# sdat2/mSWE-GNN

Measured on AMD Instinct MI355X. Metric: mesh-nodes x rollout-steps / sec (fine-scale nodes); fp32 max-abs err vs CPU ref, higher is better.
Workload: dtype f32

## Files before the change

mswe-gnn_amd/csrc/engine.h:

```cpp
#pragma once
#include <hip/hip_runtime.h>
#include <stdint.h>
#include <algorithm>

#include "graph_build.h"

namespace msw {

constexpr int kMaxLayers = 4;
constexpr int kWaves = 4;
constexpr int kRowsPerBlock = kRowsPerWave * kWaves;
constexpr int kXcds = 8, kCusPerXcd = 32;

struct LayerDev {
  int tin, tout;
  int a_off, b_off;
  int act;
  float slope;
};
struct MlpDev {
  int n;
  LayerDev l[kMaxLayers];
};

// ... 121 lines not shown
  const float* skip;
  float* out;
  int last;
  Epilogue epi;
  int coop;
  int stagger;
  int wdirect;
  int* step_inc;
  const EdgeChunk* chunks; int nchunks;
  PoolFuse pool;
};

struct HopArgs {
  Common c;
  WReg reg;
  int max_blocks;
  int fit_blocks;
  int n0;
  const LaneRec* recs; int ntiles;
  const float* s;
  const float* xs;
  const float* in;
  float* out;
  int filt_a;
  int grad, upwind;
  int last;
  Epilogue epi;
  int coop;
  int split;
  int rows;
  int nrows;
  const int* rptr;
  const int2* redge;
};


struct PoolArgs {
  Common c;
  WReg reg;
  int max_blocks;
  int fit_blocks;
  int n0, ns;
  int rows;
  int ntiles;
  const PoolRec* recs;
  const LaneRec* erecs;
  int rtiles, etiles;
  const int* child;
  const float* in;
  const float* xs;
  NpDesc np;
  int coop;
};

struct EpiArgs {
  Common c;
  WReg reg;
  int max_blocks, fit_blocks;
  int n0, ns, ntiles;
  const float* in;
  const float* xs;
  float* out;
  Epilogue epi;
};

struct DecodeArgs {
  Common c;
// ... 30 lines not shown
constexpr size_t eh_lds_bytes(int floats) {
  return (size_t)((floats + kChunk - 1) / kChunk * kChunk) * sizeof(float);
}
template <int NT>
constexpr int edge_coop_lds_cap(int pw, int fuse) {
  if constexpr (NT == 4) {
    return 160 * 1024 - (kWaves / pw) * (kRowsPerWave * (48 * NT + 4) * 4 + 2 * kRowsPerWave * (32 * NT + 4) * 4);
  } else {
    const int st = kWaves * kRowsPerWave * (48 * NT + 4) * 4 + (kWaves / 2) * 2 * kRowsPerWave * (32 * NT + 4) * 4;
    const int ps = fuse ? (kWaves / 2) * kRowsPerWave * (48 * NT + 4) * 4 : 0;
    return 160 * 1024 - st - ps;
  }
}
int set_error(int code, const char* msg);

hipError_t launch_set_slots(const SlotArgs& a, hipStream_t st);
hipError_t launch_set_io(RolloutIO* dst, const RolloutIO& v, hipStream_t st);
hipError_t launch_init_state(const InitArgs& a, hipStream_t st);
hipError_t launch_copy_rows(const float* src, const int* srows, float* dst, const int* drows, int n, int width,
                            hipStream_t st);

struct Pick {
  const void* fn;
  char name[40];
  int err;
  int grid;
  int waves;
  int pack;
  size_t lds;
  long units;
  int per_wg;
};

static inline int cdiv(long a, long b) { return (int)((a + b - 1) / b); }

template <class A>
static inline bool tile_loop(const A& a) {
  return a.fit_blocks > 0 && a.max_blocks > 0 && cdiv(a.ntiles, kWaves) > a.fit_blocks;
}

template <class A>
static inline dim3 xcd_grid(A& b, long g) {
  b.c.xcd = 0;
  for (int k = 1; k <= b.c.xcd_max && k < kXcds; k *= 2)
    if (g <= (long)kCusPerXcd * k) {
      b.c.xcd = k;
      return dim3((unsigned)(cdiv(g, k) * kXcds));
    }
  return dim3((unsigned)g);
}

template <class A>
static inline hipError_t launch_pick(const Pick& p, const A& a, hipStream_t st) {
  if (p.err) return (hipError_t)p.err;
  if (!p.fn) return hipSuccess;
  A b = a;
  const dim3 grid = p.pack ? xcd_grid(b, p.grid) : dim3((unsigned)p.grid);
  if (!p.pack) b.c.xcd = 0;
  void* args[] = {&b};
  return hipLaunchKernel(p.fn, grid, dim3(64 * p.waves), args, p.lds, st);
}

enum Family { K_ENCODE, K_ENCODE_COOP, K_EDGE_HOP, K_EDGE_COOP, K_EDGE_MLP, K_HOP, K_HOP_ROWS, K_HOP_SPLIT,
              K_HOP_COOP, K_POOL_ROWS, K_POOL_EDGE, K_EPI, K_DECODE, K_FAMILIES };
struct VariantKey {
  int family;
  int prelu = 0;
  int last = 0;
  int loop = 0;
  int waves = 0;
  int fuse = 0;
  int dec = 0;
  int stream = 0;
};

template <int NT> Pick pick_encode(const EncodeArgs& a);
template <int NT> Pick pick_edge_hop(const EdgeHopArgs& a);
template <int NT> Pick pick_edge_mlp(const EdgeHopArgs& a);
template <int NT> Pick pick_hop(const HopArgs& a);
template <int NT> Pick pick_pool(const PoolArgs& a);
template <int NT> Pick pick_epi(const EpiArgs& a);
template <int NT> Pick pick_decode(const DecodeArgs& a);
template <int NT> hipError_t prepare_kernels();
template <int NT> int resident_blocks(const VariantKey& k, int floats);
template <int NT> hipError_t launch_rowmlp(const RowMlpArgs& a, hipStream_t st);

}
```

mswe-gnn_amd/csrc/graph_build.h:

```cpp
#pragma once
#include <stdint.h>

#include <algorithm>
#include <string>
#include <vector>

#include "../../include/mswegnn.h"
#include "tiling.h"

namespace msw {

constexpr int kRowsPerWave = 16;
constexpr int kMaxScales = 8;
constexpr int kPoolInline = 4;

struct I2 {
  int x, y;
};

struct TileRange {
  int node0, nnode, edge0, nedge;
};
struct LaneRec {
  int src;
// ... 18 lines not shown
  int ntiles = 0, nchunks = 0;
  std::vector<LaneRec> recs;
  std::vector<EdgeChunk> chunks;
  std::vector<int> porig;
  std::vector<int> rptr;
  std::vector<I2> redge;
};
struct HostLevel {
  int I = 0;
  std::vector<PoolRec> pool_recs;
  std::vector<LaneRec> pool_erecs;
  int pool_etiles = 0;
  std::vector<int> pool_child;
  std::vector<PoolSlot> pool_slots;
  std::vector<LaneRec> un_recs;
  int un_ntiles = 0;
  std::vector<I2> parent_slots;
};
struct HostGraph {
  int N = 0, Npad = 0;
  int64_t E = 0;
  std::vector<int> perm, iperm;
  std::vector<HostScale> sc;
  std::vector<HostLevel> lv;
};

struct XchPeer {
  int peer, roff, rcount, soff, scount;
};
struct HostXchScale {
  std::vector<int> recv_rows, send_rows;
  std::vector<XchPeer> peers;
};

inline void csr_build(int nkeys, const std::vector<int>& key, std::vector<int>& rowptr, std::vector<int>& order) {
  rowptr.assign(nkeys + 1, 0);
  for (int k : key) rowptr[k + 1]++;
  for (int i = 0; i < nkeys; ++i) rowptr[i + 1] += rowptr[i];
  std::vector<int> pos(rowptr.begin(), rowptr.end() - 1);
  order.assign(key.size(), 0);
  for (size_t e = 0; e < key.size(); ++e) order[pos[key[e]]++] = (int)e;
}

inline int build_tiles(const std::vector<int>& rowptr, std::vector<TileRange>& out, std::string& err) {
  out.clear();
  const int ns = (int)rowptr.size() - 1;
  int a = 0;
  while (a < ns) {
    int b = a, edges = 0;
    while (b < ns && b - a < kRowsPerWave) {
      const int d = rowptr[b + 1] - rowptr[b];
      if (d > kRowsPerWave) {
        err = "node with more than 16 in-edges";
        return MSW_ERR_UNSUPPORTED;
      }
      if (edges + d > kRowsPerWave) break;
      edges += d;
      ++b;
    }
    out.push_back(TileRange{a, b - a, rowptr[a], edges});
    a = b;
  }
  return MSW_OK;
}

inline std::vector<LaneRec> make_recs(const std::vector<int>& rowptr, const std::vector<int>& src, int n0,
// ... 258 lines not shown
```

mswe-gnn_amd/csrc/kernels/k_hop.h:

```cpp
#pragma once

template <int NT>
struct HopRows {
  Lanes L;
  f32x4 os[NT], sv[NT], inn[NT];
  EpiPre<NT> pre;
};
template <int NT, bool LAST>
__device__ __forceinline__ void hop_gather(HopRows<NT>& r, const HopArgs& a, const LaneRec& rec, int tile, int j,
                                           int g) {
  constexpr int F = 16 * NT;
  r.L = lanes_of(rec, tile, j, a.n0);
  load_row<NT>(r.os, a.in + r.L.sr * F, g);
  load_row<NT>(r.sv, a.s + r.L.p * F, g);
  load_row<NT>(r.inn, a.in + r.L.n * F, g);
  if constexpr (LAST) epi_prefetch<NT>(r.pre, a.epi, a.c, a.xs, r.L.n, g);
}
template <int NT, bool LAST>
__device__ __forceinline__ void hop_load(HopRows<NT>& r, const HopArgs& a, int tile, int j, int g) {
  hop_gather<NT, LAST>(r, a, load_rec(a.recs, tile, j), tile, j, g);
}
#define MSW_ARGS_HOP(a) \
  (a).c.xcd, (a).ntiles, (a).recs, (a).n0, (a).in, (a).s, (a).out, (a).c.W, (a).filt_a, (a).grad, (a).upwind
#define MSW_ARGS_HOP_LAST(a) \
// ... 86 lines not shown
      int t1 = tile + stride;
      LaneRec rn = load_rec(a.recs, t1 < a.ntiles ? t1 : tile, j);
      for (;;) {
        const int ln = opaque_lane(), gg = ln >> 4, jj = ln & 15;
        const bool more = t1 < a.ntiles;
        HopRows<NT> qn;
        if (more) {
          hop_gather<NT, LAST>(qn, a, rn, t1, jj, gg);
          const int t2 = t1 + stride;
          rn = load_rec(a.recs, t2 < a.ntiles ? t2 : t1, jj);
        }
        f32x4 res[NT];
        core(q, jj, ln, gg, res);
        finish(res, q, ln, gg);
        if (!more) break;
        q = qn;
        t1 += stride;
      }
    }
  }
  MSW_MARK(c, 9);
}

constexpr int kRowHopWaves = 8;
constexpr int kRowDc = 3;
template <int NT>
__global__ __launch_bounds__(64 * kRowHopWaves) void k_hop_rows(HopArgs a) {
#pragma clang fp contract(off)
  constexpr int F = 16 * NT;
  constexpr int DC = NT >= 4 ? 2 : kRowDc;
  [[maybe_unused]] const int lane = threadIdx.x & 63;
  const int w = wave_id();
  const int stride = gridDim.x * kRowHopWaves;
  MSW_PIN(stride, a.nrows, a.rptr, a.redge, a.n0, a.in, a.s, a.out, a.c.W, a.filt_a, a.grad, a.upwind);
  const int ntile = (a.nrows + kRowsPerWave - 1) / kRowsPerWave;
  f32x4 wf[NT][NT];
  load_filter<NT>(wf, a.c.W, a.filt_a, lane);
  for (int tile = blockIdx.x * kRowHopWaves + w; tile < ntile; tile += stride) {
    const int ln = opaque_lane(), g = ln >> 4, j = ln & 15;
    const int k = tile * kRowsPerWave + j;
    const bool valid = k < a.nrows;
    const int kc = valid ? k : 0;
    const int q0 = a.rptr[kc], q1 = valid ? a.rptr[kc + 1] : q0;
    const size_t n = (size_t)a.n0 + kc;
    f32x4 od[NT];
    load_row<NT>(od, a.in + n * F, g);
    const int deg = q1 - q0;
    int dmax = deg;
#pragma unroll
    for (int o = 1; o < 64; o <<= 1) dmax = max(dmax, __shfl_xor(dmax, o));
    float rd = 0.f;
#pragma unroll
    for (int t = 0; t < NT; ++t) rd += hsum(od[t]);
    const bool zd = row_sum(rd) != 0.f;
    f32x4 agg[NT];
#pragma unroll
    for (int t = 0; t < NT; ++t) agg[t] = zero4();
    for (int q = 0; q < dmax; q += DC) {
      int2 e[DC];
#pragma unroll
      for (int u = 0; u < DC; ++u)
        e[u] = q + u < deg ? a.redge[q0 + q + u] : int2{(int)n, 0};
      f32x4 os[DC][NT], sv[DC][NT];
#pragma unroll
      for (int u = 0; u < DC; ++u) {
        load_row<NT>(os[u], a.in + (size_t)e[u].x * F, g);
        load_row<NT>(sv[u], a.s + (size_t)e[u].y * F, g);
      }
#pragma unroll
      for (int u = 0; u < DC; ++u) {
        float rs = 0.f;
#pragma unroll
        for (int t = 0; t < NT; ++t) rs += hsum(os[u][t]);
        const bool act = (row_sum(rs) != 0.f) || zd;
        const bool has = q + u < deg;
#pragma unroll
        for (int t = 0; t < NT; ++t) {
          f32x4 gv;
          if (a.grad) {
            gv = od[t] - os[u][t];
            if (a.upwind) {
              gv.x = gv.x < 0.f ? 0.f : gv.x; gv.y = gv.y < 0.f ? 0.f : gv.y;
              gv.z = gv.z < 0.f ? 0.f : gv.z; gv.w = gv.w < 0.f ? 0.f : gv.w;
            }
          } else {
            gv = os[u][t];
          }
          const f32x4 m = act ? gv * sv[u][t] : zero4();
          const f32x4 sum = agg[t] + m;
          agg[t] = has ? sum : agg[t];
        }
      }
    }
    f32x4 res[NT];
#pragma unroll
    for (int t = 0; t < NT; ++t) res[t] = od[t];
    apply_filter_regs<NT>(res, agg, a.filt_a, wf);
    if (valid) store_row<NT, true>(a.out + n * F, res, NT, g);
  }
}

template <int NT>
__global__ __launch_bounds__(kBlock) void k_hop_split(HopArgs a) {
#pragma clang fp contract(off)
  constexpr int F = 16 * NT, TH = NT / 2, G = kWaves / 2;
  constexpr int XS = 16 * TH + 4;
  __shared__ __attribute__((aligned(16))) float slab_all[G][2][kRowsPerWave][XS];
  __shared__ __attribute__((aligned(16))) float hx[G][2][2 * TH][64];
  __shared__ __attribute__((aligned(16))) f32x4 ax[G][NT][64];
  const int lane = threadIdx.x & 63, g = lane >> 4, j = lane & 15, w = wave_id();
  const int grp = w / 2, r = w % 2, t0 = r * TH;
  MSW_PIN(MSW_ARGS_HOP(a));
  const int xb = logical_block(a.c);
  if (xb < 0) return;
  const int tile = xb * G + grp;
  const bool live = tile < a.ntiles;
  MSW_MARK(a.c, 0);
  const Lanes L = lanes_of(load_rec(a.recs, live ? tile : 0, j), live ? tile : 0, j, a.n0);
  f32x4 os[TH], sv[TH], inn[TH];
#pragma unroll
  for (int t = 0; t < TH; ++t) {
    const int off = 16 * (t0 + t) + 4 * g;
    os[t] = ld4(a.in + L.sr * F + off);
    sv[t] = ld4(a.s + L.p * F + off);
    inn[t] = ld4(a.in + L.n * F + off);
  }
  f32x4 wf[TH][NT];
  {
    const int fa = a.filt_a >= 0 ? a.filt_a : 0;
#pragma unroll
    for (int to = 0; to < TH; ++to)
#pragma unroll
// ... 206 lines not shown
```

mswe-gnn_amd/csrc/kernels/k_launch.h:

```cpp
#pragma once

template <int NT>
hipError_t prepare_kernels() {
  std::set<const void*> done;
  hipError_t e = hipSuccess;
  for_each_key([&](const VariantKey& k) {
    const Variant v = variant_of<NT>(k);
    if (e == hipSuccess && v.fn && v.lds_cap && done.insert(v.fn).second)
      e = hipFuncSetAttribute(v.fn, hipFuncAttributeMaxDynamicSharedMemorySize, v.lds_cap);
  });
  return e;
}

template <int NT>
hipError_t launch_rowmlp(const RowMlpArgs& a, hipStream_t st) {
  if (a.R <= 0) return hipSuccess;
  if (a.mode == 1)
    hipLaunchKernelGGL((k_rowmlp<NT, 1>), dim3(cdiv(a.R, kRowsPerBlock)), dim3(kBlock), 0, st, a);
  else
    hipLaunchKernelGGL((k_rowmlp<NT, 0>), dim3(cdiv(a.R, kRowsPerBlock)), dim3(kBlock), 0, st, a);
  return hipGetLastError();
}

template <int NT>
int resident_blocks(const VariantKey& k, int floats) {
  const Variant v = variant_of<NT>(k);
  int per_cu = 0, dev = 0, cus = 0;
  if (!v.fn) return 0;
  const size_t dyn = variant_lds<NT>(v, floats);
  if (dyn > 160 * 1024) return 0;
  if (hipOccupancyMaxActiveBlocksPerMultiprocessor(&per_cu, v.fn, 64 * v.waves, dyn) != hipSuccess)
    return 0;
  if (hipGetDevice(&dev) != hipSuccess || hipDeviceGetAttribute(&cus, hipDeviceAttributeMultiprocessorCount, dev) != hipSuccess)
    return 0;
  return per_cu > 0 ? per_cu * cus : 0;
}

#define MSW_INSTANTIATE(NT)                                                       \
  template hipError_t prepare_kernels<NT>();                                      \
  template int resident_blocks<NT>(const VariantKey&, int);                       \
  template Pick pick_encode<NT>(const EncodeArgs&);                               \
  template Pick pick_edge_hop<NT>(const EdgeHopArgs&);                            \
  template Pick pick_edge_mlp<NT>(const EdgeHopArgs&);                            \
  template Pick pick_hop<NT>(const HopArgs&);                                     \
  template Pick pick_pool<NT>(const PoolArgs&);                                   \
  template Pick pick_epi<NT>(const EpiArgs&);                                     \
  template Pick pick_decode<NT>(const DecodeArgs&);                               \
  template hipError_t launch_rowmlp<NT>(const RowMlpArgs&, hipStream_t);
```

mswe-gnn_amd/csrc/kernels/k_pick.h:

```cpp
#pragma once

template <int NT>
constexpr size_t lds_bytes(int floats) {
  return kStaged<NT> ? (size_t)((floats + kChunk - 1) / kChunk * kChunk) * sizeof(float) : 0;
}

template <class A>
static inline int tile_grid(const A& a) {
  return tile_loop(a) ? a.max_blocks : cdiv(a.ntiles, kWaves);
}

enum LdsRule { LDS_NONE, LDS_STAGED, LDS_EDGE_HOP };
struct Variant {
  const void* fn;
  int waves;
  int lds;
  int lds_cap;
};
template <int NT>
static inline size_t variant_lds(const Variant& v, int floats) {
  return v.lds == LDS_EDGE_HOP ? eh_lds_bytes(floats) : v.lds == LDS_STAGED ? lds_bytes<NT>(floats) : 0;
}

template <class F>
// ... 21 lines not shown
            k.dec ? act((const void*)k_encode_coop<NT, 1, true, NT>, (const void*)k_encode_coop<NT, -1, true, NT>)
                  : act((const void*)k_encode_coop<NT, 1, false, NT>, (const void*)k_encode_coop<NT, -1, false, NT>);
        return {f, enc_coop_waves<NT>(), LDS_STAGED, mx(enc_coop_waves<NT>())};
      }
      return none;
    case K_EDGE_HOP:
      return by_flag(k.loop, [&](auto lp) {
        return by_flag(k.last, [&](auto ls) {
          constexpr bool L = decltype(lp)::value;
          constexpr int LS = decltype(ls)::value;
          return Variant{act((const void*)k_edge_hop<NT, 1, L, LS>, (const void*)k_edge_hop<NT, -1, L, LS>),
                         edge_waves<NT, L, LS>(), LDS_EDGE_HOP, mx(edge_waves<NT, L, LS>())};
        });
      });
    case K_EDGE_COOP: {
      if (k.waves != 2 && !(NT == 4 && k.waves == 4)) return none;
      const void* f = edge_coop_kernel<NT>(k.prelu, k.last, k.waves, k.fuse);
      return {f, kWaves, LDS_EDGE_HOP, f ? edge_coop_lds_cap<NT>(k.waves, k.fuse) : 0};
    }
    case K_EDGE_MLP:
      return {act((const void*)k_edge_mlp<NT, 1>, (const void*)k_edge_mlp<NT, -1>), kMlpWaves, LDS_EDGE_HOP, 160 * 1024};
    case K_HOP:
      return by_flag(k.loop, [&](auto lp) {
        constexpr bool L = decltype(lp)::value;
        const void* f = !k.last ? (const void*)k_hop<NT, 1, false, L>
                                : act((const void*)k_hop<NT, 1, true, L>, (const void*)k_hop<NT, -1, true, L>);
        return Variant{f, hop_waves<NT, L>(), LDS_STAGED, k.last ? mx(hop_waves<NT, L>()) : 0};
      });
    case K_HOP_ROWS: return {(const void*)k_hop_rows<NT>, kRowHopWaves, LDS_NONE, 0};
    case K_HOP_SPLIT:
      if constexpr (NT >= 2) return {(const void*)k_hop_split<NT>, kWaves, LDS_NONE, 0};
      return none;
    case K_HOP_COOP: return {hop_coop_kernel<NT>(k.prelu), kWaves, LDS_STAGED, mx(kWaves)};
    case K_POOL_ROWS:
      return by_flag(k.loop, [&](auto lp) {
        constexpr bool L = decltype(lp)::value;
        return Variant{(const void*)k_pool<NT, L>, waves_of<NT, L>(), LDS_STAGED, mx(waves_of<NT, L>())};
      });
    case K_POOL_EDGE:
      if (k.waves <= 1) return {(const void*)k_pool_edge<NT>, kWaves, LDS_STAGED, mx(kWaves)};
      if constexpr (NT >= 2) {
        if (k.waves == NT) return {(const void*)k_pool_edge<NT, NT>, kWaves, LDS_STAGED, mx(kWaves)};
        if (k.waves == 2 * NT) return {(const void*)k_pool_edge<NT, 2 * NT, 2 * NT>, 2 * NT, LDS_STAGED, mx(2 * NT)};
      }
      return none;
    case K_EPI:
      return by_flag(k.loop, [&](auto lp) {
        constexpr bool L = decltype(lp)::value;
        return Variant{act((const void*)k_epi<NT, 1, L>, (const void*)k_epi<NT, -1, L>), waves_of<NT, L>(), LDS_STAGED,
                       mx(waves_of<NT, L>())};
      });
    case K_DECODE:
      return {act((const void*)k_decode_fwd<NT, 1>, (const void*)k_decode_fwd<NT, -1>), kWaves, LDS_NONE, 0};
  }
  return none;
}

template <class F>
static inline void for_each_key(F&& f) {
  for (int family = 0; family < K_FAMILIES; ++family)
    for (int bits = 0; bits < 32; ++bits)
      for (int waves : {1, 2, 4, 8})
        for (int fuse = 0; fuse < 3; ++fuse)
          f(VariantKey{family, bits & 1, bits >> 1 & 1, bits >> 2 & 1, waves, fuse, bits >> 3 & 1, bits >> 4 & 1});
}

// ... 64 lines not shown
                         a.ntiles, kWaves / a.coop);
  }
  if (a.pool.slots || a.pool.parent) return pick_invalid();
  const bool loop = tile_loop(a);
  const Variant v = variant_of<NT>({K_EDGE_HOP, a.c.prelu, a.last, loop});
  return pick_make<NT>(v, pick_name(nm, "edge_hop", {{loop, "loop"}, {last, "last"}, {!last, "first"}}), tile_grid(a),
                       !loop, loop ? a.reg.len : a.reg_nf, a.ntiles, v.waves);
}

template <int NT>
Pick pick_hop(const HopArgs& a) {
  if (a.ntiles <= 0) return Pick{};
  char nm[40];
  if (a.coop > 1 && a.last)
    return pick_make<NT>(variant_of<NT>({K_HOP_COOP, a.c.prelu, 1, 0, a.coop}), "hop coop",
                         cdiv((long)a.ntiles * a.coop, kWaves), 1, a.reg.len, a.ntiles, kWaves / a.coop);
  if (a.rows && !a.last) {
    const int nt = cdiv(a.nrows, kRowsPerWave);
    const int grid = a.max_blocks > 0 ? std::min(a.max_blocks, cdiv(nt, kRowHopWaves)) : cdiv(nt, kRowHopWaves);
    return pick_make<NT>(variant_of<NT>({K_HOP_ROWS}), "hop rows", grid, 0, 0, nt, kRowHopWaves);
  }
  if constexpr (NT >= 2) {
    if (a.split && !a.last)
      return pick_make<NT>(variant_of<NT>({K_HOP_SPLIT}), "hop split", cdiv((long)a.ntiles * 2, kWaves), 1, 0,
                           a.ntiles, kWaves / 2);
  }
  const bool loop = tile_loop(a), last = a.last != 0;
  const Variant v = variant_of<NT>({K_HOP, a.c.prelu, last, loop});
  return pick_make<NT>(v, pick_name(nm, "hop", {{loop, "loop"}, {last, "last"}, {!last, "mid"}}), tile_grid(a), !loop,
                       last ? a.reg.len : 0, a.ntiles, v.waves);
}

template <int NT>
Pick pick_pool(const PoolArgs& a) {
  if (a.ntiles <= 0) return Pick{};
  if (!a.rows) {
    if constexpr (NT >= 2) {
      if (a.coop == 2 * NT)
        return pick_make<NT>(variant_of<NT>({K_POOL_EDGE, 0, 0, 0, 2 * NT}), "pool edge wide", a.ntiles, 1, a.reg.len,
                             a.ntiles, 1);
      if (a.coop == NT)
        return pick_make<NT>(variant_of<NT>({K_POOL_EDGE, 0, 0, 0, NT}), "pool edge coop",
                             cdiv((long)a.ntiles * NT, kWaves), 1, a.reg.len, a.ntiles, kWaves / NT);
    }
    return pick_make<NT>(variant_of<NT>({K_POOL_EDGE}), "pool edge", cdiv(a.ntiles, kWaves), 1, a.reg.len, a.ntiles,
                         kWaves);
  }
  const bool loop = tile_loop(a);
  const Variant v = variant_of<NT>({K_POOL_ROWS, 0, 0, loop});
  return pick_make<NT>(v, loop ? "pool rows loop" : "pool rows", tile_grid(a), !loop, a.reg.len, a.ntiles, v.waves);
}

template <int NT>
Pick pick_epi(const EpiArgs& a) {
  if (a.ntiles <= 0) return Pick{};
  const bool loop = tile_loop(a);
  const Variant v = variant_of<NT>({K_EPI, a.c.prelu, 1, loop});
  return pick_make<NT>(v, loop ? "epi loop" : "epi", tile_grid(a), !loop, a.reg.len, a.ntiles, v.waves);
}

template <int NT>
Pick pick_decode(const DecodeArgs& a) {
  if (a.Npad <= 0) return Pick{};
  const int n = cdiv(a.Npad, kRowsPerBlock);
  return pick_make<NT>(variant_of<NT>({K_DECODE, a.c.prelu}), "decode", n, 0, 0, n, 1);
}
// ... 1 lines not shown
```

mswe-gnn_amd/csrc/plan.hip:

```cpp
#include <atomic>
#include <cmath>
#include <cstdio>
#include <dlfcn.h>
#include <rccl/rccl.h>

#include <cstdlib>
#include <cstring>
#include <map>
#include <memory>
#include <numeric>
#include <string>
#include <type_traits>
#include <vector>

#include "../../include/mswegnn.h"
#include "tiling.h"
#include "engine.h"

using namespace msw;

namespace {

thread_local std::string g_err;

// ... 99 lines not shown

template <class T>
int upload(T** p, const std::vector<T>& v, int64_t& counter) {
  int rc = dalloc(p, v.size(), counter);
  if (rc) return rc;
  if (!v.empty()) HIP_TRY(hipMemcpy(*p, v.data(), v.size() * sizeof(T), hipMemcpyHostToDevice));
  return MSW_OK;
}

template <class F>
auto with_nt(int NT, F&& f) {
  switch (NT) {
    case 1: return f(std::integral_constant<int, 1>{});
    case 2: return f(std::integral_constant<int, 2>{});
    default: return f(std::integral_constant<int, 4>{});
  }
}

hipError_t rowmlp_dispatch(int NT, const RowMlpArgs& ra, hipStream_t st = nullptr) {
  return with_nt(NT, [&](auto nt) { return launch_rowmlp<nt>(ra, st); });
}

}

struct ScaleCSR {
  int n0 = 0, ns = 0;
  int E = 0;
  LaneRec* recs = nullptr;
  int ntiles = 0;
  EdgeChunk* chunks = nullptr;
  int nchunks = 0;
  int* rptr = nullptr;
  int2* redge = nullptr;

  std::vector<int> porig;
  std::vector<LaneRec> hrecs;
};

struct LevelMaps {
  int I = 0;
  PoolRec* pool_recs = nullptr;
  LaneRec* pool_erecs = nullptr;
  int pool_etiles = 0;
  int* pool_child = nullptr;
  PoolSlot* pool_slots = nullptr;
  int2* parent_slots = nullptr;
  LaneRec* un_recs = nullptr;
  int un_ntiles = 0;
};

struct Proc {
  int scale = 0;
  int K = 0, normalize = 1, with_filter = 1, with_gradient = 1, upwind = 0;
  int h1t = 1;
  int a_u = -1, a_v = -1, a_o = -1;
  int a_vu = -1;
  float* Pe = nullptr;
  int b1_off = -1;
  int act1 = 0;
  float slope1 = 0.f;
  MlpDev rest{};
  std::vector<int> filt;
  int prelu = 0;
  int par = 0;
};

// ... 14 lines not shown
    void* h = RTLD_DEFAULT;
    if (!dlsym(h, "ncclSend")) {
      h = dlopen("librccl.so.1", RTLD_NOW | RTLD_GLOBAL);
      if (!h) return a;
    }
    a.getUniqueId = (decltype(a.getUniqueId))dlsym(h, "ncclGetUniqueId");
    a.commInitRank = (decltype(a.commInitRank))dlsym(h, "ncclCommInitRank");
    a.commDestroy = (decltype(a.commDestroy))dlsym(h, "ncclCommDestroy");
    a.groupStart = (decltype(a.groupStart))dlsym(h, "ncclGroupStart");
    a.groupEnd = (decltype(a.groupEnd))dlsym(h, "ncclGroupEnd");
    a.send = (decltype(a.send))dlsym(h, "ncclSend");
    a.recv = (decltype(a.recv))dlsym(h, "ncclRecv");
    a.errStr = (decltype(a.errStr))dlsym(h, "ncclGetErrorString");
    a.ok = a.getUniqueId && a.commInitRank && a.commDestroy && a.groupStart && a.groupEnd && a.send &&
           a.recv && a.errStr;
    return a;
  }();
  return api;
}

enum LaunchKind { L_ENCODE, L_EDGE_HOP, L_HOP, L_POOL, L_EXCHANGE, L_EPI, L_EDGE_MLP, L_DECODE };

enum BufId { B_U0, B_U1, B_O0, B_O1, B_T0, B_T1 };
struct ExchangeArgs {
  Common c;
  int scale;
  int nbuf;
  int buf[2];
  int width[2];
};
struct Launch {
  int kind;
  int scale;
  union {
    EncodeArgs enc;
    EdgeHopArgs eh;
    HopArgs hop;
    PoolArgs pool;
    ExchangeArgs xch;
    EpiArgs ep;
    DecodeArgs dec;
  };
  Launch() { memset((void*)this, 0, sizeof(*this)); }
  template <class L, class F>
  static decltype(auto) visit(L& l, F&& f) {
    switch (l.kind) {
      case L_ENCODE: return f(l.enc);
      case L_EDGE_HOP:
      case L_EDGE_MLP: return f(l.eh);
      case L_HOP: return f(l.hop);
      case L_EXCHANGE: return f(l.xch);
      case L_EPI: return f(l.ep);
      case L_DECODE: return f(l.dec);
      default: return f(l.pool);
    }
  }
  Common& common() {
    return visit(*this, [](auto& a) -> Common& { return a.c; });
  }
  const Common& common() const {
    return visit(*this, [](const auto& a) -> const Common& { return a.c; });
  }
};

struct Knobs {
  int split_edge_mlp = -1;
  int pool_fuse = 1;
  int unpool_fuse = 1;
  int defer_decode = -1;
  int hop_rows = -1;
  int coop2_direct = 1;
  int coop2_f64 = 1;
  int enc_coop = -1;
  int eh_loop = 0;
  int hop_split = -1;
  int pool_wide = 1;
  int tile_pack = 1;
  int xcd_max = 1;
  int coop_waves = -1;
  int epi_split_tiles = -1;
  int trace_encode = 0;
  int grid_cap = 0;
};
inline Knobs knobs_from_env() {
  Knobs k;
  const struct { const char* name; int* v; } tab[] = {
      {"MSW_SPLIT_EDGE_MLP", &k.split_edge_mlp}, {"MSW_POOL_FUSE", &k.pool_fuse},
      {"MSW_UNPOOL_FUSE", &k.unpool_fuse}, {"MSW_DEFER_DECODE", &k.defer_decode}, {"MSW_HOP_ROWS", &k.hop_rows},
      {"MSW_COOP2_DIRECT", &k.coop2_direct}, {"MSW_COOP2_F64", &k.coop2_f64}, {"MSW_ENC_COOP", &k.enc_coop},
      {"MSW_EH_LOOP", &k.eh_loop},
      {"MSW_HOP_SPLIT", &k.hop_split}, {"MSW_POOL_WIDE", &k.pool_wide}, {"MSW_TILE_PACK", &k.tile_pack},
      {"MSW_XCD_MAX", &k.xcd_max}, {"MSW_COOP_WAVES", &k.coop_waves},
      {"MSW_EPI_SPLIT_TILES", &k.epi_split_tiles}, {"MSW_TRACE_ENCODE", &k.trace_encode},
      {"MSW_GRID_CAP", &k.grid_cap}};
  for (const auto& t : tab)
    if (const char* e = getenv(t.name)) *t.v = atoi(e);
  return k;
}

struct msw_plan {
  int device = 0;
  int F = 32, Fp = 32;
  int model_type = 0, NT = 2, S = 1, p = 3, nnf = 8, dyn = 6, nstat_raw = 2;
  int with_wl = 1, skip = 1;
  int N = 0, Npad = 0;
  int64_t E = 0;
  std::vector<int> perm, iperm;
  std::vector<ScaleCSR> sc;
  std::vector<LevelMaps> lv;
  std::vector<Proc> procs, unpools;
  MlpDev stat{}, dynm{}, dec{}, edge_enc{};
  int gnn_act = 0;
  float gnn_slope = 0.f;
  int resw_off = -1;
  int prelu = 0;
  Blob blob;
  float* dW = nullptr;
  int* perm_d = nullptr;
  int* bc_slot_d = nullptr;
  float* zrow_d = nullptr;
  std::vector<int> bc_rows_set;
  RolloutIO* io_d = nullptr;
  std::vector<RowMlpArgs> edge_jobs;
  float *X = nullptr, *xs = nullptr, *xd0 = nullptr;
// ... 578 lines not shown
      if (!a.last) continue;
      RegionBuilder R(P->blob, 0);
      rl.epi(R, a.epi);
      a.reg = R.done();
      reg = &a.reg;
    } else {
      PoolArgs& a = L.pool;
      RegionBuilder R(P->blob, 0);
      rl.np(R, a.np);
      a.reg = R.done();
      reg = &a.reg;
    }
    if (reg) tot = (reg->len + 255) / 256 * 256;
    if (tot > kMaxRegionFloats)
      return fail(MSW_ERR_UNSUPPORTED, "weights of one launch exceed the LDS budget (" + std::to_string(tot * 4) + " B)");
  }
  return MSW_OK;
}

int resident_of(const msw_plan* P, const VariantKey& k, int floats) {
  const int r = with_nt(P->NT, [&](auto nt) { return resident_blocks<nt>(k, floats); });
  return P->kn.grid_cap > 0 ? std::min(r, P->kn.grid_cap) : r;
}
template <class A>
void caps(const msw_plan* P, A& a, VariantKey k, int floats) {
  k.loop = 1;
  a.max_blocks = resident_of(P, k, floats);
  k.loop = 0;
  a.fit_blocks = resident_of(P, k, floats);
}
constexpr int kHopLoopTiles = 65536;
constexpr int kRowHopMinTiles = kHopLoopTiles;
bool row_hops_forced(const msw_plan* P) { return P->kn.hop_rows == 2; }
constexpr long kEncCoopWaves = 4096;
void cap_encode(const msw_plan* P, EncodeArgs& a) {
  a.max_blocks = resident_of(P, {K_ENCODE, a.c.prelu}, a.lds_floats);
  bool coop = P->NT == 4 && (long)(a.Npad / kRowsPerWave) * P->NT <= kEncCoopWaves;
  if (P->kn.enc_coop >= 0) coop = P->NT >= 2 && P->kn.enc_coop != 0;
  a.coop = coop ? P->NT : 0;
  a.stream = !a.coop && !a.dec.on && a.max_blocks > 0 && a.Npad / kRowsPerBlock > a.max_blocks;
}
void cap_edge_mlp(const msw_plan* P, EdgeHopArgs& a) {
  a.stagger = kMlpStagger;
  a.max_blocks = resident_of(P, {K_EDGE_MLP, a.c.prelu}, a.reg.len);
}
void cap_edge_hop(const msw_plan* P, EdgeHopArgs& a) {
  a.max_blocks = resident_of(P, {K_EDGE_HOP, a.c.prelu, a.last, 1}, a.reg.len);
  a.fit_blocks = resident_of(P, {K_EDGE_HOP, a.c.prelu, a.last, 0}, a.reg_nf);
  if (P->kn.eh_loop && a.max_blocks > 0 && a.ntiles > kWaves) a.fit_blocks = 1;
  const bool loop = tile_loop(a);
  const bool epi_ok = !a.last || (!a.epi.dec.on && a.epi.uu_a < 0);
  const int pw = P->NT == 2 ? 2 : P->NT == 4 ? 4 : 0;
  const int coop_fit = pw ? resident_of(P, {K_EDGE_COOP, a.c.prelu, a.last, 0, pw}, a.reg_nf) : 0;
  a.coop = (pw && !loop && epi_ok && P->coop_waves > 0 && (long)pw * a.ntiles <= P->coop_waves &&
            (pw * a.ntiles + kWaves - 1) / kWaves <= coop_fit) ? pw : 0;
  if ((a.pool.slots || a.pool.parent) && P->NT == 2) a.coop = 2;
  const int c2 = P->kn.coop2_f64;
  if (c2 == 2 && a.coop == 4) a.coop = 0;
  a.wdirect = 0;
  if (P->NT == 4 && !a.coop && !loop && epi_ok && P->coop_waves > 0 && 2L * a.ntiles <= P->coop_waves && c2) {
    const int need = (2 * a.ntiles + kWaves - 1) / kWaves;
    const int wd = P->kn.coop2_direct;
    const VariantKey two{K_EDGE_COOP, a.c.prelu, a.last, 0, 2};
    if (need <= resident_of(P, two, a.reg_nf)) {
      a.coop = 2;
      a.wdirect = wd == 2 && a.reg.len > 0;
    } else if (wd != 0 && a.reg.len > 0 && need <= resident_of(P, two, 0)) {
      a.coop = 2;
      a.wdirect = 1;
    }
  }
  if ((a.pool.slots || a.pool.parent) && !a.coop) a.coop = 2;
}
void cap_hop(const msw_plan* P, HopArgs& h) {
  caps(P, h, {K_HOP, h.c.prelu, h.last}, h.reg.len);
  if (h.ntiles < kHopLoopTiles && P->kn.grid_cap <= 0) h.max_blocks = 0;
  {
    bool sp = P->NT == 4 && h.max_blocks == 0;
    if (P->kn.hop_split >= 0) sp = P->kn.hop_split != 0;
    h.split = (sp && P->NT >= 2 && !h.last) ? 1 : 0;
  }
  h.rows = 0;
  if (P->kn.hop_rows != 0 && !h.last && (tile_loop(h) || row_hops_forced(P)) && h.rptr && h.redge) {
    h.rows = 1;
    h.split = 0;
    h.max_blocks = resident_of(P, {K_HOP_ROWS}, 0);
  }
  const int pw = P->NT >= 2 ? P->NT : 0;
  h.coop = 0;
  if (h.last && pw && !tile_loop(h) && P->coop_waves > 0 && (long)pw * h.ntiles <= P->coop_waves &&
      (pw * h.ntiles + kWaves - 1) / kWaves <= resident_of(P, {K_HOP_COOP, h.c.prelu, 1, 0, pw}, h.reg.len))
    h.coop = pw;
}
void cap_pool(const msw_plan* P, PoolArgs& a) {
  const int fe = resident_of(P, {K_POOL_EDGE}, a.reg.len);
  a.rows = !(fe > 0 && (a.etiles + kWaves - 1) / kWaves <= fe);
  a.ntiles = a.rows ? a.rtiles : a.etiles;
  caps(P, a, {K_POOL_ROWS}, a.reg.len);
  const int pw = P->NT >= 2 ? P->NT : 0;
  a.coop = (!a.rows && pw && P->coop_waves > 0 && (long)pw * a.etiles <= P->coop_waves &&
            (pw * a.etiles + kWaves - 1) / kWaves <= fe) ? pw : 0;
  const bool wide = P->kn.pool_wide != 0;
  if (wide && pw && a.coop == pw && a.np.h1t == 2 * pw) {
    const int f8 = resident_of(P, {K_POOL_EDGE, 0, 0, 0, 2 * pw}, a.reg.len);
    if (f8 > 0 && a.etiles <= f8) a.coop = 2 * pw;
  }
}
void set_grid_cap(const msw_plan* P, Launch& L) {
  if (L.kind != L_HOP && L.kind != L_EDGE_HOP && L.kind != L_POOL && L.kind != L_EPI) L.common().xcd_max = 0;
  switch (L.kind) {
    case L_ENCODE: return cap_encode(P, L.enc);
    case L_EDGE_MLP: return cap_edge_mlp(P, L.eh);
    case L_EDGE_HOP: return cap_edge_hop(P, L.eh);
    case L_HOP: return cap_hop(P, L.hop);
    case L_EPI: return caps(P, L.ep, {K_EPI, L.ep.c.prelu, 1}, L.ep.reg.len);
    case L_POOL: return cap_pool(P, L.pool);
    default: return;
  }
}

const Launch* lds_overflow(const msw_plan* P) {
  for (const auto* q : {&P->sched_fwd, &P->sched_roll})
    for (const Launch& L : *q) {
      if (L.kind != L_EDGE_HOP || !(L.eh.coop == 2 || L.eh.coop == 4) || L.eh.wdirect) continue;
      const int fuse = L.eh.pool.slots ? 1 : L.eh.pool.parent ? 2 : 0;
      const int cap = with_nt(P->NT, [&](auto nt) { return edge_coop_lds_cap<nt>(L.eh.coop, fuse); });
      if (eh_lds_bytes(L.eh.reg_nf) > (size_t)cap) return &L;
    }
  return nullptr;
}

template <int NT>
Pick pick_one(const Launch& L) {
  switch (L.kind) {
    case L_ENCODE: return pick_encode<NT>(L.enc);
    case L_EDGE_HOP: return pick_edge_hop<NT>(L.eh);
    case L_EDGE_MLP: return pick_edge_mlp<NT>(L.eh);
    case L_HOP: return pick_hop<NT>(L.hop);
    case L_POOL: return pick_pool<NT>(L.pool);
    case L_EPI: return pick_epi<NT>(L.ep);
    case L_DECODE: return pick_decode<NT>(L.dec);
    default: return Pick{};
  }
}
Pick pick_one(const msw_plan* P, const Launch& L) {
  return with_nt(P->NT, [&](auto nt) { return pick_one<nt>(L); });
}
hipError_t launch_one(const msw_plan* P, const Launch& L, hipStream_t st) {
  if (L.kind == L_EXCHANGE) return hipErrorInvalidValue;
  return Launch::visit(L, [&](const auto& args) { return launch_pick(pick_one(P, L), args, st); });
}

float* buf_of(msw_plan* P, int id) {
  switch (id) {
    case B_U0: return P->U[0];
    case B_U1: return P->U[1];
    case B_O0: return P->O[0];
    case B_O1: return P->O[1];
    case B_T0: return P->T[0];
    default: return P->T[1];
  }
}

int rccl_exchange(msw_plan* P, const ExchangeArgs& a, hipStream_t st) {
  const msw_plan::XchScale& X = P->xch[a.scale];
  if (!P->comm) return fail(MSW_ERR_INVALID, "partitioned plan without a transport (msw_plan_set_comm)");
  RcclApi& r = rccl();
  for (int b = 0; b < a.nbuf; ++b) {
    float* buf = buf_of(P, a.buf[b]);
    const int w = a.width[b];
    HIP_TRY(launch_copy_rows(buf, X.send_rows, P->xsend, nullptr, X.nsend, w, st));
    ncclResult_t e = r.groupStart();
    for (const auto& pe : X.peers) {
      if (e == ncclSuccess && pe.scount > 0 &&
          (e = r.send(P->xsend + (size_t)pe.soff * w, (size_t)pe.scount * w, ncclFloat32, pe.peer, P->comm, st)) ==
              ncclSuccess)
        ++P->rccl_calls;
      if (e == ncclSuccess && pe.rcount > 0 &&
          (e = r.recv(P->xrecv + (size_t)pe.roff * w, (size_t)pe.rcount * w, ncclFloat32, pe.peer, P->comm, st)) ==
              ncclSuccess)
        ++P->rccl_calls;
    }
// ... 274 lines not shown
    if ((rc = build_proc(P.get(), m->unpool[i], P->S - 2 - (int)i, true, P->unpools[i]))) return rc;
  }
  P->prelu = all_prelu(m->static_encoder) & all_prelu(m->dynamic_encoder) & all_prelu(m->decoder);

  if ((rc = pupload(P.get(), &P->perm_d, P->perm))) return rc;
  if ((rc = pupload(P.get(), &P->zrow_d, std::vector<float>(kZeroRow, 0.f)))) return rc;
  std::vector<int> minus1(Npad, -1);
  if ((rc = pupload(P.get(), &P->bc_slot_d, minus1))) return rc;
  if ((rc = palloc(P.get(), &P->io_d, 1))) return rc;
  HIP_TRY(hipMemset(P->io_d, 0, sizeof(RolloutIO)));
  int Emax = 1;
  for (auto& c : P->sc) Emax = std::max(Emax, c.ntiles * kRowsPerWave);
  const size_t NF = (size_t)Npad * Fp;
  const size_t NH = (size_t)Npad * 16 * P->h1t_max;
  float** bufs[] = {&P->xs, &P->xd0, &P->O[0], &P->O[1], &P->T[0], &P->T[1], &P->xdown, &P->xup, &P->xgnn};
  for (float** b : bufs) {
    if ((rc = palloc(P.get(), b, NF))) return rc;
    HIP_TRY(hipMemset(*b, 0, NF * sizeof(float)));
  }
  float** hbufs[] = {&P->U[0], &P->V[0], &P->U[1], &P->V[1], &P->Uu, &P->Vu};
  for (float** b : hbufs) {
    if ((rc = palloc(P.get(), b, NH))) return rc;
    HIP_TRY(hipMemset(*b, 0, NH * sizeof(float)));
  }
  if ((rc = palloc(P.get(), &P->s, (size_t)Emax * Fp))) return rc;
  if ((rc = palloc(P.get(), &P->X, (size_t)Npad * P->nnf))) return rc;
  HIP_TRY(hipMemset(P->X, 0, (size_t)Npad * P->nnf * sizeof(float)));
  if (P->E > 0)
    for (Proc& pr : P->procs)
      if ((rc = palloc(P.get(), &pr.Pe, (size_t)std::max(P->sc[pr.scale].ntiles * kRowsPerWave, 1) * 16 * pr.h1t)))
        return rc;

  HIP_TRY(with_nt(P->NT, [](auto nt) { return prepare_kernels<nt>(); }));
  const size_t blob0 = P->blob.h.size();
  for (;;) {
    sched_step(P.get(), P->sched_fwd, false);
    sched_step(P.get(), P->sched_roll, true);
    const bool mlp_only = P->NT > 2;
    if ((rc = relocate(P.get(), P->sched_fwd, mlp_only)) || (rc = relocate(P.get(), P->sched_roll, mlp_only)))
      return rc;
    for (auto* q : {&P->sched_fwd, &P->sched_roll})
      for (Launch& L : *q) set_grid_cap(P.get(), L);
    const Launch* bad = lds_overflow(P.get());
    if (!bad) break;
    if (P->no_fuse || !(bad->eh.pool.slots || bad->eh.pool.parent))
      return fail(MSW_ERR_UNSUPPORTED, "weights of a cooperative edge hop exceed its LDS budget (" +
                                           std::to_string(eh_lds_bytes(bad->eh.reg_nf)) + " B)");
    P->no_fuse = 1;
    P->blob.h.resize(blob0);
  }
  P->blob.alloc(256);
  if ((rc = pupload(P.get(), &P->dW, P->blob.h))) return rc;
  for (auto* q : {&P->sched_fwd, &P->sched_roll})
    for (Launch& L : *q) L.common().W = P->dW;

  if (P->E > 0) {
    std::vector<int64_t> sbase(P->S + 1, 0);
    for (int s = 0; s < P->S; ++s) sbase[s + 1] = sbase[s] + (int64_t)P->sc[s].ntiles * kRowsPerWave;
    const int64_t E = sbase[P->S];
    std::vector<float> ea((size_t)std::max<int64_t>(E, 1) * ef_raw, 0.f);
    for (int s = 0; s < P->S; ++s)
      for (size_t q = 0; q < P->sc[s].porig.size(); ++q)
        if (P->sc[s].porig[q] >= 0)
          for (int f = 0; f < ef_raw; ++f)
            ea[(size_t)(sbase[s] + q) * ef_raw + f] = g->edge_attr[(size_t)P->sc[s].porig[q] * ef_raw + f];
    float* ea_d = nullptr;
// ... 439 lines not shown
```

Before: 54.32 million.

## Add dense per-row hop kernel with inline edge records for small scales

Adds a dense hop kernel that assigns one row per lane group and reads up to four incoming edges from a packed per-row record, falling back to a CSR list for higher degree. It is selected by default for small scales that fit in one resident wave each, bypassing the tiled/coop hop paths. It aims to cut per-tile indirection and launch work on coarse scales, at the cost of extra device buffers and single-wave blocks with possibly low occupancy. It also makes row-hop non-temporal stores conditional on an encode-residency heuristic.

```diff
diff --git a/mswe-gnn_amd/csrc/engine.h b/mswe-gnn_amd/csrc/engine.h
--- a/mswe-gnn_amd/csrc/engine.h
+++ b/mswe-gnn_amd/csrc/engine.h
@@ -177,7 +177,36 @@
   int nrows;
   const int* rptr;
   const int2* redge;
-};
+  int stream;
+};
+
+struct DenseHopArgs {
+  Common c;
+  int n0, nrows;
+  const DenseRec* recs;
+  const float* in;
+  const float* s;
+  float* out;
+  int filt_a;
+  int grad, upwind;
+  const int* rptr;
+  const int2* redge;
+  int post_act; float post_slope;
+};
+static inline bool bare_epilogue(const Epilogue& e) {
+  return e.np.a_u < 0 && e.np.a_v < 0 && e.np.a_o < 0 && e.uu_a < 0 && !e.dec.on;
+}
+static inline DenseHopArgs dense_args(const HopArgs& a, const DenseRec* recs, const int* rptr, const int2* redge) {
+  DenseHopArgs d{};
+  d.c = a.c;
+  d.n0 = a.n0; d.nrows = a.nrows; d.recs = recs;
+  d.in = a.in; d.s = a.s; d.out = a.out;
+  d.filt_a = a.filt_a; d.grad = a.grad; d.upwind = a.upwind;
+  d.rptr = rptr; d.redge = redge;
+  d.post_act = a.last ? a.epi.post_act : 0;
+  d.post_slope = a.epi.post_slope;
+  return d;
+}
 
 
 struct PoolArgs {
@@ -274,6 +303,7 @@
   int per_wg;
 };
 
+
 static inline int cdiv(long a, long b) { return (int)((a + b - 1) / b); }
 
 template <class A>
@@ -304,7 +334,7 @@
 }
 
 enum Family { K_ENCODE, K_ENCODE_COOP, K_EDGE_HOP, K_EDGE_COOP, K_EDGE_MLP, K_HOP, K_HOP_ROWS, K_HOP_SPLIT,
-              K_HOP_COOP, K_POOL_ROWS, K_POOL_EDGE, K_EPI, K_DECODE, K_FAMILIES };
+              K_HOP_COOP, K_HOP_DENSE, K_POOL_ROWS, K_POOL_EDGE, K_EPI, K_DECODE, K_FAMILIES };
 struct VariantKey {
   int family;
   int prelu = 0;
@@ -320,6 +350,7 @@
 template <int NT> Pick pick_edge_hop(const EdgeHopArgs& a);
 template <int NT> Pick pick_edge_mlp(const EdgeHopArgs& a);
 template <int NT> Pick pick_hop(const HopArgs& a);
+template <int NT> Pick pick_hop_dense(const HopArgs& a);
 template <int NT> Pick pick_pool(const PoolArgs& a);
 template <int NT> Pick pick_epi(const EpiArgs& a);
 template <int NT> Pick pick_decode(const DecodeArgs& a);
diff --git a/mswe-gnn_amd/csrc/graph_build.h b/mswe-gnn_amd/csrc/graph_build.h
--- a/mswe-gnn_amd/csrc/graph_build.h
+++ b/mswe-gnn_amd/csrc/graph_build.h
@@ -74,6 +74,43 @@
   std::vector<int> recv_rows, send_rows;
   std::vector<XchPeer> peers;
 };
+
+constexpr int kDenseInline = 4;
+struct alignas(16) DenseRec {
+  I2 e[kDenseInline];
+};
+struct HostDense {
+  std::vector<DenseRec> recs;
+  std::vector<int> rptr;
+  std::vector<I2> redge;
+};
+inline HostDense build_dense(const std::vector<LaneRec>& recs, int n0, int ns) {
+  HostDense d;
+  const int padded = (ns + kRowsPerWave - 1) / kRowsPerWave * kRowsPerWave;
+  d.recs.assign((size_t)std::max(padded, kRowsPerWave), DenseRec{{{-1, 0}, {-1, 0}, {-1, 0}, {-1, 0}}});
+  std::vector<int> first(ns, 0), deg(ns, 0);
+  for (size_t t = 0; t * kRowsPerWave < recs.size(); ++t)
+    for (int j = 0; j < kRowsPerWave; ++j) {
+      const LaneRec& r = recs[t * kRowsPerWave + j];
+      if (r.n < 0) continue;
+      const int k = r.n - n0;
+      if (k < 0 || k >= ns) continue;
+      first[k] = (int)(t * kRowsPerWave) + (r.q & 255);
+      deg[k] = (r.q >> 8) - (r.q & 255);
+    }
+  d.rptr.assign(ns + 1, 0);
+  for (int k = 0; k < ns; ++k) d.rptr[k + 1] = d.rptr[k] + deg[k];
+  d.redge.assign(std::max(d.rptr[ns], 1), I2{n0, 0});
+  for (int k = 0; k < ns; ++k)
+    for (int q = 0; q < deg[k]; ++q) {
+      const I2 e{recs[first[k] + q].src, first[k] + q};
+      d.redge[d.rptr[k] + q] = e;
+      if (q < kDenseInline) d.recs[k].e[q] = e;
+    }
+  for (int k = 0; k < ns; ++k)
+    if (deg[k] > kDenseInline) d.recs[k].e[kDenseInline - 1].y = ~d.recs[k].e[kDenseInline - 1].y;
+  return d;
+}
 
 inline void csr_build(int nkeys, const std::vector<int>& key, std::vector<int>& rowptr, std::vector<int>& order) {
   rowptr.assign(nkeys + 1, 0);
diff --git a/mswe-gnn_amd/csrc/kernels/k_hop.h b/mswe-gnn_amd/csrc/kernels/k_hop.h
--- a/mswe-gnn_amd/csrc/kernels/k_hop.h
+++ b/mswe-gnn_amd/csrc/kernels/k_hop.h
@@ -142,7 +142,7 @@
   [[maybe_unused]] const int lane = threadIdx.x & 63;
   const int w = wave_id();
   const int stride = gridDim.x * kRowHopWaves;
-  MSW_PIN(stride, a.nrows, a.rptr, a.redge, a.n0, a.in, a.s, a.out, a.c.W, a.filt_a, a.grad, a.upwind);
+  MSW_PIN(stride, a.nrows, a.rptr, a.redge, a.n0, a.in, a.s, a.out, a.c.W, a.filt_a, a.grad, a.upwind, a.stream);
   const int ntile = (a.nrows + kRowsPerWave - 1) / kRowsPerWave;
   f32x4 wf[NT][NT];
   load_filter<NT>(wf, a.c.W, a.filt_a, lane);
@@ -206,8 +206,111 @@
 #pragma unroll
     for (int t = 0; t < NT; ++t) res[t] = od[t];
     apply_filter_regs<NT>(res, agg, a.filt_a, wf);
-    if (valid) store_row<NT, true>(a.out + n * F, res, NT, g);
-  }
+    if (valid) {
+      if (a.stream)
+        store_row<NT, true>(a.out + n * F, res, NT, g);
+      else
+        store_row<NT>(a.out + n * F, res, NT, g);
+    }
+  }
+}
+
+template <int NT, int ACT, bool LAST>
+__global__ __launch_bounds__(64) void k_hop_dense(DenseHopArgs a) {
+#pragma clang fp contract(off)
+  static_assert(NT <= 2, "4 x 2 NT + NT row loads per lane: F <= 32");
+  constexpr int F = 16 * NT, DC = kDenseInline;
+  const int lane = threadIdx.x & 63, g = lane >> 4, j = lane & 15;
+  MSW_PIN(a.c.xcd, a.nrows, a.recs, a.n0, a.in, a.s, a.out, a.c.W, a.filt_a, a.grad, a.upwind);
+  const int xb = logical_block(a.c);
+  if (xb < 0) return;
+  if (xb * kRowsPerWave >= a.nrows) return;
+  const int k = xb * kRowsPerWave + j;
+  MSW_MARK(a.c, 0);
+  f32x4 wf[NT][NT];
+  load_filter<NT>(wf, a.c.W, a.filt_a, lane);
+  const bool valid = k < a.nrows;
+  const int4 r0 = reinterpret_cast<const int4*>(a.recs)[2 * (size_t)k];
+  const int4 r1 = reinterpret_cast<const int4*>(a.recs)[2 * (size_t)k + 1];
+  const size_t n = (size_t)a.n0 + k;
+  f32x4 od[NT];
+  load_row<NT>(od, a.in + n * F, g);
+  MSW_MARK(a.c, 1);
+  const bool more = r1.z >= 0 && r1.w < 0;
+  const int src[DC] = {r0.x, r0.z, r1.x, r1.z};
+  const int slot[DC] = {r0.y, r0.w, r1.y, r1.w < 0 ? ~r1.w : r1.w};
+  f32x4 os[DC][NT], sv[DC][NT];
+  const size_t own_s = src[0] >= 0 ? (size_t)slot[0] : 0;
+  auto fetch = [&](int u) {
+    const bool has = src[u] >= 0;
+    load_row<NT>(os[u], a.in + (has ? (size_t)src[u] : n) * F, g);
+    load_row<NT>(sv[u], a.s + (has ? (size_t)slot[u] : own_s) * F, g);
+  };
+#pragma unroll
+  for (int u = 0; u < DC - 1; ++u) fetch(u);
+  const bool four = __any(src[DC - 1] >= 0);
+#pragma unroll
+  for (int t = 0; t < NT; ++t) os[DC - 1][t] = sv[DC - 1][t] = zero4();
+  if (four) fetch(DC - 1);
+  MSW_MARK(a.c, 4);
+  float rd = 0.f;
+#pragma unroll
+  for (int t = 0; t < NT; ++t) rd += hsum(od[t]);
+  const bool zd = row_sum(rd) != 0.f;
+  f32x4 agg[NT];
+#pragma unroll
+  for (int t = 0; t < NT; ++t) agg[t] = zero4();
+  auto edge = [&](const f32x4(&so)[NT], const f32x4(&se)[NT], bool has) {
+    float rs = 0.f;
+#pragma unroll
+    for (int t = 0; t < NT; ++t) rs += hsum(so[t]);
+    const bool act = (row_sum(rs) != 0.f) || zd;
+#pragma unroll
+    for (int t = 0; t < NT; ++t) {
+      f32x4 gv;
+      if (a.grad) {
+        gv = od[t] - so[t];
+        if (a.upwind) {
+          gv.x = gv.x < 0.f ? 0.f : gv.x; gv.y = gv.y < 0.f ? 0.f : gv.y;
+          gv.z = gv.z < 0.f ? 0.f : gv.z; gv.w = gv.w < 0.f ? 0.f : gv.w;
+        }
+      } else {
+        gv = so[t];
+      }
+      const f32x4 m = act ? gv * se[t] : zero4();
+      const f32x4 sum = agg[t] + m;
+      agg[t] = has ? sum : agg[t];
+    }
+  };
+#pragma unroll
+  for (int u = 0; u < DC - 1; ++u) edge(os[u], sv[u], src[u] >= 0);
+  if (four) edge(os[DC - 1], sv[DC - 1], src[DC - 1] >= 0);
+  if (__any(more)) {
+    const int q0 = a.rptr[valid ? k : 0];
+    const int deg = more ? a.rptr[k + 1] - q0 : 0;
+    for (int q = DC; __any(q < deg); ++q) {
+      const bool has = q < deg;
+      const int2 e = has ? a.redge[q0 + q] : int2{(int)n, 0};
+      f32x4 so[NT], se[NT];
+      load_row<NT>(so, a.in + (size_t)e.x * F, g);
+      load_row<NT>(se, a.s + (size_t)e.y * F, g);
+      edge(so, se, has);
+    }
+  }
+  MSW_MARK(a.c, 7);
+  f32x4 res[NT];
+#pragma unroll
+  for (int t = 0; t < NT; ++t) res[t] = od[t];
+  apply_filter_regs<NT>(res, agg, a.filt_a, wf);
+  MSW_MARK(a.c, 8);
+  if constexpr (LAST) {
+    if (a.post_act) {
+      act_tiles<-1, NT>(res, a.post_act, a.post_slope);
+      mask_pad<ACT, NT>(res, a.c.fl, g);
+    }
+  }
+  if (valid) store_row<NT>(a.out + n * F, res, NT, g);
+  MSW_MARK(a.c, 9);
 }
 
 template <int NT>
diff --git a/mswe-gnn_amd/csrc/kernels/k_launch.h b/mswe-gnn_amd/csrc/kernels/k_launch.h
--- a/mswe-gnn_amd/csrc/kernels/k_launch.h
+++ b/mswe-gnn_amd/csrc/kernels/k_launch.h
@@ -43,6 +43,7 @@
   template Pick pick_edge_hop<NT>(const EdgeHopArgs&);                            \
   template Pick pick_edge_mlp<NT>(const EdgeHopArgs&);                            \
   template Pick pick_hop<NT>(const HopArgs&);                                     \
+  template Pick pick_hop_dense<NT>(const HopArgs&);                               \
   template Pick pick_pool<NT>(const PoolArgs&);                                   \
   template Pick pick_epi<NT>(const EpiArgs&);                                     \
   template Pick pick_decode<NT>(const DecodeArgs&);                               \
diff --git a/mswe-gnn_amd/csrc/kernels/k_pick.h b/mswe-gnn_amd/csrc/kernels/k_pick.h
--- a/mswe-gnn_amd/csrc/kernels/k_pick.h
+++ b/mswe-gnn_amd/csrc/kernels/k_pick.h
@@ -77,6 +77,13 @@
       if constexpr (NT >= 2) return {(const void*)k_hop_split<NT>, kWaves, LDS_NONE, 0};
       return none;
     case K_HOP_COOP: return {hop_coop_kernel<NT>(k.prelu), kWaves, LDS_STAGED, mx(kWaves)};
+    case K_HOP_DENSE:
+      if constexpr (NT <= 2) {
+        const void* f = !k.last ? (const void*)k_hop_dense<NT, 1, false>
+                                : act((const void*)k_hop_dense<NT, 1, true>, (const void*)k_hop_dense<NT, -1, true>);
+        return {f, 1, LDS_NONE, 0};
+      }
+      return none;
     case K_POOL_ROWS:
       return by_flag(k.loop, [&](auto lp) {
         constexpr bool L = decltype(lp)::value;
@@ -207,6 +214,15 @@
 }
 
 template <int NT>
+Pick pick_hop_dense(const HopArgs& a) {
+  if (a.nrows <= 0) return Pick{};
+  char nm[40];
+  const int nt = cdiv(a.nrows, kRowsPerWave);
+  return pick_make<NT>(variant_of<NT>({K_HOP_DENSE, a.c.prelu, a.last != 0}),
+                       pick_name(nm, "hop dense", {{a.last != 0, "last"}}), nt, 1, 0, nt, 1);
+}
+
+template <int NT>
 Pick pick_pool(const PoolArgs& a) {
   if (a.ntiles <= 0) return Pick{};
   if (!a.rows) {
diff --git a/mswe-gnn_amd/csrc/plan.hip b/mswe-gnn_amd/csrc/plan.hip
--- a/mswe-gnn_amd/csrc/plan.hip
+++ b/mswe-gnn_amd/csrc/plan.hip
@@ -155,6 +155,9 @@
   int nchunks = 0;
   int* rptr = nullptr;
   int2* redge = nullptr;
+  DenseRec* drecs = nullptr;
+  int* dptr = nullptr;
+  int2* dedge = nullptr;
 
   std::vector<int> porig;
   std::vector<LaneRec> hrecs;
@@ -235,6 +238,7 @@
 struct Launch {
   int kind;
   int scale;
+  int dense;
   union {
     EncodeArgs enc;
     EdgeHopArgs eh;
@@ -277,6 +281,7 @@
   int enc_coop = -1;
   int eh_loop = 0;
   int hop_split = -1;
+  int hop_dense = 1;
   int pool_wide = 1;
   int tile_pack = 1;
   int xcd_max = 1;
@@ -292,7 +297,7 @@
       {"MSW_UNPOOL_FUSE", &k.unpool_fuse}, {"MSW_DEFER_DECODE", &k.defer_decode}, {"MSW_HOP_ROWS", &k.hop_rows},
       {"MSW_COOP2_DIRECT", &k.coop2_direct}, {"MSW_COOP2_F64", &k.coop2_f64}, {"MSW_ENC_COOP", &k.enc_coop},
       {"MSW_EH_LOOP", &k.eh_loop},
-      {"MSW_HOP_SPLIT", &k.hop_split}, {"MSW_POOL_WIDE", &k.pool_wide}, {"MSW_TILE_PACK", &k.tile_pack},
+      {"MSW_HOP_SPLIT", &k.hop_split}, {"MSW_HOP_DENSE", &k.hop_dense}, {"MSW_POOL_WIDE", &k.pool_wide}, {"MSW_TILE_PACK", &k.tile_pack},
       {"MSW_XCD_MAX", &k.xcd_max}, {"MSW_COOP_WAVES", &k.coop_waves},
       {"MSW_EPI_SPLIT_TILES", &k.epi_split_tiles}, {"MSW_TRACE_ENCODE", &k.trace_encode},
       {"MSW_GRID_CAP", &k.grid_cap}};
@@ -937,6 +942,24 @@
 constexpr int kHopLoopTiles = 65536;
 constexpr int kRowHopMinTiles = kHopLoopTiles;
 bool row_hops_forced(const msw_plan* P) { return P->kn.hop_rows == 2; }
+constexpr int kDenseMaxTiles = 2048;
+bool dense_hops(const msw_plan* P, const ScaleCSR& c) {
+  if (P->NT > 2 || P->part_rank >= 0 || P->kn.grid_cap > 0 || P->kn.hop_dense == 0) return false;
+  if (row_hops_forced(P) || (P->kn.hop_split > 0 && P->NT >= 2)) return false;
+  const int nt = cdiv(c.ns, kRowsPerWave);
+  if (nt <= 0 || c.ntiles <= 0 || nt > kDenseMaxTiles) return false;
+  return nt <= resident_of(P, {K_HOP_DENSE, P->prelu, 1}, 0);
+}
+int upload_dense(msw_plan* P) {
+  for (ScaleCSR& c : P->sc) {
+    if (!dense_hops(P, c)) continue;
+    const HostDense d = build_dense(c.hrecs, c.n0, c.ns);
+    int rc;
+    if ((rc = pupload(P, &c.drecs, d.recs)) || (rc = pupload(P, &c.dptr, d.rptr)) || (rc = pupload(P, &c.dedge, d.redge)))
+      return rc;
+  }
+  return MSW_OK;
+}
 constexpr long kEncCoopWaves = 4096;
 void cap_encode(const msw_plan* P, EncodeArgs& a) {
   a.max_blocks = resident_of(P, {K_ENCODE, a.c.prelu}, a.lds_floats);
@@ -977,7 +1000,8 @@
   }
   if ((a.pool.slots || a.pool.parent) && !a.coop) a.coop = 2;
 }
-void cap_hop(const msw_plan* P, HopArgs& h) {
+void cap_hop(const msw_plan* P, Launch& L) {
+  HopArgs& h = L.hop;
   caps(P, h, {K_HOP, h.c.prelu, h.last}, h.reg.len);
   if (h.ntiles < kHopLoopTiles && P->kn.grid_cap <= 0) h.max_blocks = 0;
   {
@@ -990,10 +1014,17 @@
     h.rows = 1;
     h.split = 0;
     h.max_blocks = resident_of(P, {K_HOP_ROWS}, 0);
-  }
+    int enc_floats = 0;
+    for (const Launch& E : P->sched_fwd)
+      if (E.kind == L_ENCODE) enc_floats = E.enc.lds_floats;
+    const int enc_fit = resident_of(P, {K_ENCODE, P->prelu}, enc_floats);
+    h.stream = enc_fit > 0 && P->Npad / kRowsPerBlock > enc_fit;
+  }
+  L.dense = P->sc[L.scale].drecs && !h.rows && !tile_loop(h) && (!h.last || bare_epilogue(h.epi));
+  if (L.dense) h.split = 0;
   const int pw = P->NT >= 2 ? P->NT : 0;
   h.coop = 0;
-  if (h.last && pw && !tile_loop(h) && P->coop_waves > 0 && (long)pw * h.ntiles <= P->coop_waves &&
+  if (h.last && !L.dense && pw && !tile_loop(h) && P->coop_waves > 0 && (long)pw * h.ntiles <= P->coop_waves &&
       (pw * h.ntiles + kWaves - 1) / kWaves <= resident_of(P, {K_HOP_COOP, h.c.prelu, 1, 0, pw}, h.reg.len))
     h.coop = pw;
 }
@@ -1017,7 +1048,7 @@
     case L_ENCODE: return cap_encode(P, L.enc);
     case L_EDGE_MLP: return cap_edge_mlp(P, L.eh);
     case L_EDGE_HOP: return cap_edge_hop(P, L.eh);
-    case L_HOP: return cap_hop(P, L.hop);
+    case L_HOP: return cap_hop(P, L);
     case L_EPI: return caps(P, L.ep, {K_EPI, L.ep.c.prelu, 1}, L.ep.reg.len);
     case L_POOL: return cap_pool(P, L.pool);
     default: return;
@@ -1041,7 +1072,7 @@
     case L_ENCODE: return pick_encode<NT>(L.enc);
     case L_EDGE_HOP: return pick_edge_hop<NT>(L.eh);
     case L_EDGE_MLP: return pick_edge_mlp<NT>(L.eh);
-    case L_HOP: return pick_hop<NT>(L.hop);
+    case L_HOP: return L.dense ? pick_hop_dense<NT>(L.hop) : pick_hop<NT>(L.hop);
     case L_POOL: return pick_pool<NT>(L.pool);
     case L_EPI: return pick_epi<NT>(L.ep);
     case L_DECODE: return pick_decode<NT>(L.dec);
@@ -1053,6 +1084,10 @@
 }
 hipError_t launch_one(const msw_plan* P, const Launch& L, hipStream_t st) {
   if (L.kind == L_EXCHANGE) return hipErrorInvalidValue;
+  if (L.kind == L_HOP && L.dense) {
+    const ScaleCSR& c = P->sc[L.scale];
+    return launch_pick(pick_one(P, L), dense_args(L.hop, c.drecs, c.dptr, c.dedge), st);
+  }
   return Launch::visit(L, [&](const auto& args) { return launch_pick(pick_one(P, L), args, st); });
 }
 
@@ -1393,6 +1428,7 @@
         return rc;
 
   HIP_TRY(with_nt(P->NT, [](auto nt) { return prepare_kernels<nt>(); }));
+  if ((rc = upload_dense(P.get()))) return rc;
   const size_t blob0 = P->blob.h.size();
   for (;;) {
     sched_step(P.get(), P->sched_fwd, false);
```

Result: faster. 54.98 million, median of 6 (+1.2%).
